# iliasam/STM32F4_SDR_GPS

Hardware: AMD Instinct MI355X
Metric: acquisition hypotheses/sec (PRN x Doppler x phase) (higher is better)
Workload: dtype u1 (MX-FP4 operands, exact f32 accumulation)

## Files before the change

### stm32f4_sdr_gps_amd/csrc/k_acq_mx.hip

```cpp
#if !defined(GPSX_LAB) && defined(MX_VARIANT_B)
#error "variants of k_acq_mx for same-box A/B timing build with -DGPSX_LAB only: tools/build_variant.sh"
#endif
#include <cstdlib>

#include "gpsx_device.hpp"
#include "gpsx_kernels.hpp"

namespace gpsx {

namespace {

typedef int v8i __attribute__((ext_vector_type(8)));
typedef int v4i __attribute__((ext_vector_type(4)));
typedef float v16f __attribute__((ext_vector_type(16)));

constexpr int kMxThreads = 512;
constexpr int kMxTiles = 4;
constexpr int kCopyDwords = 260;
constexpr int kVecDwords = 258;
constexpr int kPlaneWordsMx = 66;
constexpr u32 kScaleOne = 0x7F7F7F7Fu;
constexpr u32 kScaleA = 0x72727272u;
constexpr float kAccScale = 1.0f / 8192.0f;
constexpr float kUnscaleSq = 67108864.0f;
constexpr u32 kScaleEight = 0x82828282u;
constexpr int kPasses = 17;

struct MxShared {
  uint16_t x[1024];
  u32 d[2][514];
  u32 plane[2][16][kPlaneWordsMx];
  u32 base[2][kCopyDwords];
  u32 e8[2][2][8][kCopyDwords];
  u32 corr[2][2][2][128];
  v4i chips_a[16][2][32];
  u32 chip_t[1032];
  u32 ones[2];
  u32 t_lut[768];
  alignas(16) u32 part[8][32][2][32];
};

__device__ __forceinline__ v8i widen(v4i x) { return v8i{x.x, x.y, x.z, x.w, 0, 0, 0, 0}; }

__device__ __forceinline__ u32 lds_byte(const u32 *words, int byte_index)
{
  return (words[byte_index >> 2] >> ((byte_index & 3) * 8)) & 0xFFu;
}

__device__ __forceinline__ u32 spread8(u32 x)
{
  u32 t = (x | (x << 12)) & 0x000F000Fu;
  t = (t | (t << 6)) & 0x03030303u;
  t = (t | (t << 3)) & 0x11111111u;
  return t;
}

__device__ __forceinline__ int wrap1023(int i)
{
  i = i >= 2 * kChips ? i - 2 * kChips : i;
  return i >= kChips ? i - kChips : i;
}

__device__ __forceinline__ u32 plane_bits9(const u32 *pl, int pos)
{
  return __builtin_amdgcn_alignbit(pl[(pos >> 5) + 1], pl[pos >> 5], (u32)(pos & 31)) & 0x1FFu;
}

__device__ __forceinline__ void mx_load_block(MxShared &sh, const uint8_t *blk, int if_format, int tid)
{
  for (int i = tid; i < 1024; i += kMxThreads)
    sh.x[i] = i < kWords16 ? load_sign16(blk, i, if_format) : (uint16_t)0;
  if (tid < 2)
    sh.ones[tid] = 0;
}
__device__ void mx_wipe_block(MxShared &sh, u32 step_word, int tid, int lane)
{
  {
    const u32 *x32 = reinterpret_cast<const u32 *>(sh.x);
    u32 ones_i = 0, ones_q = 0;
    for (int w = tid; w < 514; w += kMxThreads) {
      u32 vi = 0, vq = 0;
      if (w < kWords32) {
        const u32 quad = (step_word * (u32)w) >> 30;
        vi = carrier_i(quad) ^ x32[w];
        vq = carrier_q(quad) ^ x32[w];
      }
      sh.d[0][w] = vi;
      sh.d[1][w] = vq;
      ones_i += __popc(vi);
      ones_q += __popc(vq);
    }
    ones_i = wave_sum_to_lane63(ones_i);
    ones_q = wave_sum_to_lane63(ones_q);
    if (lane == 63) {
      atomicAdd(&sh.ones[0], ones_i);
      atomicAdd(&sh.ones[1], ones_q);
    }
  }
  __syncthreads();
  if (tid < 2)
    sh.d[tid][511] = sh.d[tid][0] << 16;
  __syncthreads();
  for (int m = tid; m < 2 * 32 * 16; m += kMxThreads) {
    const int t0 = m & 15, w = (m >> 4) & 31, iq = m >> 9;
    const u32 *src = &sh.d[iq][16 * w];
    u32 bits = 0;
#pragma unroll
    for (int k = 0; k < 16; k++) {
      const u32 sk = src[k];
      bits |= ((sk >> t0) & 1u) << (2 * k);
      bits |= ((sk >> (16 + t0)) & 1u) << (2 * k + 1);
    }
    sh.plane[iq][t0][w] = bits;
  }
  __syncthreads();
  for (int m = tid; m < 2 * 16 * (kPlaneWordsMx - 32); m += kMxThreads) {
    const int w = 32 + m % (kPlaneWordsMx - 32);
    const int r = m / (kPlaneWordsMx - 32);
    const u32 *pl = sh.plane[r >> 4][r & 15];
    const int pos = 32 * w - (w >= 64 ? 2 * kChips : kChips);
    const int lo = pos >> 5;
    u32 v = __builtin_amdgcn_alignbit(lo < 31 ? pl[lo + 1] : 0u, pl[lo], (u32)(pos & 31));
    if (pos + 32 > kChips) {
      const int k = kChips - pos;
      v = (v & ((1u << k) - 1u)) | (pl[0] << k);
    }
    sh.plane[r >> 4][r & 15][w] = v;
  }
}

__device__ __forceinline__ u32 fp4_code(int v)
{
  const u32 m = (u32)(v < 0 ? -v : v);
  return ((0x0765420u >> (4u * (m > 5u ? 5u : m))) & 0xFu) | (v < 0 ? 8u : 0u);
}

__device__ void mx_fill_tables(MxShared &sh, int tid)
{
  for (int w = tid; w < 512; w += kMxThreads) {
    const u32 cur = (u32)w & 0xFFu, nxt = ((u32)w >> 1) & 0xFFu;
    const u32 plus = spread8(nxt & ~cur), minus = spread8(cur & ~nxt);
    sh.t_lut[w] = (plus << 2) | (plus << 3) | (minus << 2);
  }
  for (int x = tid; x < 256; x += kMxThreads)
    sh.t_lut[512 + x] = (spread8((u32)x) << 1) | (spread8(~(u32)x & 0xFFu) * 0xAu);
}

__device__ void mx_vector_phase1(MxShared &sh, int pass, int buf, int tid, int nthreads)
{
  const int t0 = pass - 1;
  for (int m = tid; m < 2 * kVecDwords + 2 * 128; m += nthreads) {
    if (m < 2 * kVecDwords) {
      const int iq = m >= kVecDwords, dw = m - iq * kVecDwords;
      u32 packed = 0;
      if (pass < 2) {
        const u32 *dd = sh.d[iq];
#pragma unroll
        for (int e = 0; e < 8; e++) {
          const int k = wrap1023(8 * dw + e);
          const int pos = 16 * k;
          const u32 sum = pop16(__builtin_amdgcn_alignbit(dd[(pos >> 5) + 1], dd[pos >> 5], (u32)(pos & 31)));
          const u32 code = pass == 0 ? (0xFEC0u >> (4u * (sum & 3u))) & 0xFu : (0xEDCA0u >> (4u * (sum >> 2))) & 0xFu;
          packed |= code << (4 * e);
        }
      } else {
        const u32 w = plane_bits9(sh.plane[iq][pass - 2], 8 * dw);
        packed = sh.t_lut[w];
        if (dw == 127 && t0 >= 9) {
          const u32 cur = w & 0xFFu, nxt = (w >> 1) & 0xFFu;
          const int e5 = (int)((nxt >> 5) & 1u) - (int)((cur >> 5) & 1u), e6 = (int)((nxt >> 6) & 1u) - (int)((cur >> 6) & 1u);
          packed = (packed & ~0x0FF00000u) | (fp4_code(-2 * e5 - 1) << 20) | (fp4_code(-2 * e6 + 1) << 24);
        }
      }
      sh.base[iq][dw] = packed;
    } else {
      const int mm = m - 2 * kVecDwords;
      const int iq = mm >> 7, dw = mm & 127;
      u32 ca = 0, cb = 0;
      if (pass >= 2 && t0 != 8) {
        const u32 *pl = sh.plane[iq][pass - 2];
        const u32 w = dw ? plane_bits9(pl, 8 * dw - 1) : (pl[0] << 1) & 0x1FFu;
        const u32 exist = dw == 127 ? 0x0FFFFFFFu : 0xFFFFFFFFu;
        if (t0 < 8) {
          ca = sh.t_lut[512 + (w >> 1)] & exist;
        } else {
          const u32 diff = sh.t_lut[w];
          ca = (diff ^ ((diff & 0x44444444u) << 1)) & exist;
          cb = sh.t_lut[512 + (w & 0xFFu)] & exist;
          if (dw == 0) {
            ca = (ca & ~0xFu) | ((w & 2u) ? 0x2u : 0xAu);
            cb &= ~0xFu;
          }
        }
      }
      sh.corr[buf][iq][0][dw] = ca;
      sh.corr[buf][iq][1][dw] = cb;
    }
  }
}

__device__ void mx_vector_phase2(MxShared &sh, int buf, int tid, int nthreads)
{
  for (int m = tid; m < 2 * 256; m += nthreads) {
    const int iq = m >> 8, j = m & 255;
    const u32 lo = sh.base[iq][j], hi = sh.base[iq][j + 1];
#pragma unroll
    for (int c = 0; c < 8; c++)
      sh.e8[buf][iq][c][j] = c ? __builtin_amdgcn_alignbit(hi, lo, 4u * (u32)c) : lo;
  }
}

typedef __attribute__((address_space(3))) const u32 lds_cu32;

__device__ __forceinline__ lds_cu32 *lds_opaque(const u32 *p)
{
  u32 a = (u32)(size_t)(lds_cu32 *)p;
  asm volatile("" : "+v"(a));
  return (lds_cu32 *)(size_t)a;
}
__device__ __forceinline__ v4i lds_frag(lds_cu32 *w, int dw)
{
  return v4i{(int)w[dw], (int)w[dw + 1], (int)w[dw + 2], (int)w[dw + 3]};
}

__device__ __forceinline__ u32 mx_patch_wrap(u32 packed, u32 w9, bool patch)
{
  const u32 i5 = 1u + ((w9 >> 6) & 1u) - ((w9 >> 5) & 1u), i6 = 1u + ((w9 >> 7) & 1u) - ((w9 >> 6) & 1u);
  const u32 c5 = (0xDA2u >> (4u * i5)) & 0xFu;
  const u32 c6 = (0xA25u >> (4u * i6)) & 0xFu;
  const u32 patched = (packed & ~0x0FF00000u) | (c5 << 20) | (c6 << 24);
  return patch ? patched : packed;
}

__device__ __forceinline__ void mx_vector_build(MxShared &sh, int p_vec, int tid)
{
  const int t0 = p_vec - 1, buf = p_vec & 1;
  const bool late = t0 >= 9;
  const int iq = tid >> 8, j = tid & 255, which = (tid >> 7) & 1, dwc = tid & 127;
  const u32 *pl = sh.plane[iq][p_vec - 2];
  const u32 x = __builtin_amdgcn_alignbit(pl[(j >> 2) + 1], pl[j >> 2], 8u * (u32)(j & 3));
  const int pos = dwc ? 8 * dwc - 1 : 0;
  const u32 y = __builtin_amdgcn_alignbit(pl[(pos >> 5) + 1], pl[pos >> 5], (u32)(pos & 31));
  const u32 cw = (dwc ? y : y << 1) & 0x1FFu;
  u32 lo = sh.t_lut[x & 0x1FFu], hi = sh.t_lut[(x >> 8) & 0x1FFu];
  u32 v = sh.t_lut[which ? 512u + (cw & 0xFFu) : (late ? cw : 512u + (cw >> 1))];
  if (late) {
    lo = mx_patch_wrap(lo, x & 0x1FFu, j == 127);
    hi = mx_patch_wrap(hi, (x >> 8) & 0x1FFu, j == 126);
    if (which == 0)
      v ^= (v & 0x44444444u) << 1;
    if (dwc == 0)
      v = (v & ~0xFu) | (which ? 0u : ((cw & 2u) ? 0x2u : 0xAu));
  }
  v &= dwc == 127 ? 0x0FFFFFFFu : 0xFFFFFFFFu;
  if ((which && !late) || t0 == 8)
    v = 0;
  sh.corr[buf][iq][which][dwc] = v;
  u32 *dst = &sh.e8[buf][iq][0][j];
#pragma unroll
  for (int c = 0; c < 8; c++)
    dst[c * kCopyDwords] = c ? __builtin_amdgcn_alignbit(hi, lo, 4u * (u32)c) : lo;
}

__device__ __forceinline__ void mx_vector_build_direct(MxShared &sh, int which, int t0s, u32 *e8_dst, int tid)
{
  const int iq = tid >> 8, j = tid & 255;
  const u32 *dd = sh.d[iq];
  u32 w2[2] = {0, 0};
#pragma unroll
  for (int e = 0; e < 16; e++) {
    const int k = wrap1023(8 * j + e);
    const int pos = 16 * k + t0s;
    const u32 sum = pop16(__builtin_amdgcn_alignbit(dd[(pos >> 5) + 1], dd[pos >> 5], (u32)(pos & 31)));
    const u32 code = which == 0 ? (0xFEC0u >> (4u * (sum & 3u))) & 0xFu : (0xEDCA0u >> (4u * (sum >> 2))) & 0xFu;
    w2[e >> 3] |= code << (4 * (e & 7));
  }
  u32 *dst = e8_dst + (iq * 8) * kCopyDwords + j;
#pragma unroll
  for (int c = 0; c < 8; c++)
    dst[c * kCopyDwords] = c ? __builtin_amdgcn_alignbit(w2[1], w2[0], 4u * (u32)c) : w2[0];
}

template <int S, int NT, u32 SCALE_A = kScaleA>
__device__ __forceinline__ void mx_pass_step(lds_cu32 *wi, lds_cu32 *wq, const v4i *ca, v4i (&a)[16], v4i &fi, v4i &fq,
                                             v16f (&acc)[2][NT], u32 scale_b)
{
  constexpr int kSteps = 16 + NT - 1;
  constexpr bool more = S + 1 < kSteps;
  v4i fi_next = fi, fq_next = fq;
  if constexpr (more) {
    fi_next = lds_frag(wi, 8 * (S + 1));
    fq_next = lds_frag(wq, 8 * (S + 1));
    if constexpr (S + 1 < 16)
      a[S + 1] = ca[(S + 1) * 64];
  }
  constexpr int j_lo = S - 15 > 0 ? S - 15 : 0, j_hi = S < NT - 1 ? S : NT - 1;
#pragma unroll
  for (int j = j_lo; j <= j_hi; j++) {
    acc[0][j] = __builtin_amdgcn_mfma_scale_f32_32x32x64_f8f6f4(widen(a[S - j]), widen(fi), acc[0][j], 4, 4, 0, SCALE_A, 0, scale_b);
    acc[1][j] = __builtin_amdgcn_mfma_scale_f32_32x32x64_f8f6f4(widen(a[S - j]), widen(fq), acc[1][j], 4, 4, 0, SCALE_A, 0, scale_b);
  }
  if constexpr (more) {
    __builtin_amdgcn_sched_group_barrier(0x100, S + 1 < 16 ? 5 : 4, 0);
    __builtin_amdgcn_sched_group_barrier(0x008, 2 * (j_hi - j_lo + 1), 0);
  }
  __builtin_amdgcn_sched_barrier(0);
  fi = fi_next;
  fq = fq_next;
  if constexpr (more)
    mx_pass_step<S + 1, NT, SCALE_A>(wi, wq, ca, a, fi, fq, acc, scale_b);
}

template <int S, int NT>
__device__ __forceinline__ void mx_pass_step_inplace(lds_cu32 *wi, lds_cu32 *wq, const v4i *ca, v4i (&a)[16], v4i &fi, v4i &fq,
                                                     v16f (&acc)[2][NT], u32 scale_b)
{
  constexpr int kSteps = 16 + NT - 1;
  constexpr bool more = S + 1 < kSteps;
  if constexpr (more && S + 1 < 16)
    a[S + 1] = ca[(S + 1) * 64];
  constexpr int j_lo = S - 15 > 0 ? S - 15 : 0, j_hi = S < NT - 1 ? S : NT - 1;
#pragma unroll
  for (int j = j_lo; j <= j_hi; j++)
    acc[0][j] = __builtin_amdgcn_mfma_scale_f32_32x32x64_f8f6f4(widen(a[S - j]), widen(fi), acc[0][j], 4, 4, 0, kScaleA, 0, scale_b);
  if constexpr (more)
    fi = lds_frag(wi, 8 * (S + 1));
#pragma unroll
  for (int j = j_lo; j <= j_hi; j++)
    acc[1][j] = __builtin_amdgcn_mfma_scale_f32_32x32x64_f8f6f4(widen(a[S - j]), widen(fq), acc[1][j], 4, 4, 0, kScaleA, 0, scale_b);
  if constexpr (more)
    fq = lds_frag(wq, 8 * (S + 1));
  if constexpr (more) {
    if constexpr (S + 1 < 16)
      __builtin_amdgcn_sched_group_barrier(0x100, 1, 0);
    __builtin_amdgcn_sched_group_barrier(0x008, j_hi - j_lo + 1, 0);
    __builtin_amdgcn_sched_group_barrier(0x100, 2, 0);
    __builtin_amdgcn_sched_group_barrier(0x008, j_hi - j_lo + 1, 0);
    __builtin_amdgcn_sched_group_barrier(0x100, 2, 0);
  }
  __builtin_amdgcn_sched_barrier(0);
  if constexpr (more)
    mx_pass_step_inplace<S + 1, NT>(wi, wq, ca, a, fi, fq, acc, scale_b);
}

template <int S, int NT>
__device__ __forceinline__ void mx_pass2_step(lds_cu32 *const (&w)[4], const v4i *ca, v4i (&a)[16], v4i (&f)[4], v16f (&acc)[2][NT])
{
  constexpr int kSteps = 16 + NT - 1;
  constexpr bool more = S + 1 < kSteps;
  if constexpr (more && S + 1 < 16)
    a[S + 1] = ca[(S + 1) * 64];
  constexpr int j_lo = S - 15 > 0 ? S - 15 : 0, j_hi = S < NT - 1 ? S : NT - 1;
#pragma unroll
  for (int v = 0; v < 4; v++) {
#pragma unroll
    for (int j = j_lo; j <= j_hi; j++)
      acc[v & 1][j] = __builtin_amdgcn_mfma_scale_f32_32x32x64_f8f6f4(widen(a[S - j]), widen(f[v]), acc[v & 1][j], 4, 4, 0, kScaleA, 0,
                                                                      v < 2 ? kScaleOne : kScaleEight);
    if constexpr (more)
      f[v] = lds_frag(w[v], 8 * (S + 1));
  }
  if constexpr (more) {
    if constexpr (S + 1 < 16)
      __builtin_amdgcn_sched_group_barrier(0x100, 1, 0);
#pragma unroll
    for (int v = 0; v < 4; v++) {
      __builtin_amdgcn_sched_group_barrier(0x008, j_hi - j_lo + 1, 0);
      __builtin_amdgcn_sched_group_barrier(0x100, 2, 0);
    }
  }
  __builtin_amdgcn_sched_barrier(0);
  if constexpr (more)
    mx_pass2_step<S + 1, NT>(w, ca, a, f, acc);
}
template <int NT>
__device__ __forceinline__ void mx_pass2(const MxShared &sh, int lane, int q0_tile, v16f (&acc)[2][NT], const u32 *e8_low,
                                         const u32 *e8_high)
{
  const int n = lane & 31, h = lane >> 5;
  const int off = (n & 7) * kCopyDwords + 4 * (q0_tile + h) + (n >> 3);
  lds_cu32 *const w[4] = {lds_opaque(e8_low + off), lds_opaque(e8_low + 8 * kCopyDwords + off), lds_opaque(e8_high + off),
                          lds_opaque(e8_high + 8 * kCopyDwords + off)};
  const v4i *ca = &sh.chips_a[0][h][n];
  v4i a[16];
  v4i f[4] = {lds_frag(w[0], 0), lds_frag(w[1], 0), lds_frag(w[2], 0), lds_frag(w[3], 0)};
  a[0] = ca[0];
  mx_pass2_step<0, NT>(w, ca, a, f, acc);
}

template <bool AHEAD, int NT, u32 SCALE_A = kScaleA>
__device__ __forceinline__ void mx_pass(const MxShared &sh, int buf, int lane, int q0_tile, v16f (&acc)[2][NT],
                                        u32 scale_b, v4i a_corr, bool with_corr, const u32 *e8_buf = nullptr)
{
  const int n = lane & 31, h = lane >> 5;
  const u32 *e8 = e8_buf ? e8_buf : &sh.e8[buf][0][0][0];
  lds_cu32 *wi = lds_opaque(e8 + (n & 7) * kCopyDwords + 4 * (q0_tile + h) + (n >> 3));
  lds_cu32 *wq = lds_opaque(e8 + (8 + (n & 7)) * kCopyDwords + 4 * (q0_tile + h) + (n >> 3));
  const v4i *ca = &sh.chips_a[0][h][n];
  v4i a[16];
  if constexpr (AHEAD) {
    v4i fi = lds_frag(wi, 0), fq = lds_frag(wq, 0);
    a[0] = ca[0];
    mx_pass_step<0, NT, SCALE_A>(wi, wq, ca, a, fi, fq, acc, scale_b);
  } else {
    static_assert(SCALE_A == kScaleA, "the in-place walk is the sign-only grid's");
    v4i fi = lds_frag(wi, 0), fq = lds_frag(wq, 0);
    a[0] = ca[0];
    mx_pass_step_inplace<0, NT>(wi, wq, ca, a, fi, fq, acc, scale_b);
  }
  if (with_corr) {
    lds_cu32 *cw = lds_opaque(&sh.corr[buf][0][h][4 * q0_tile + (n >> 3)]);
#pragma unroll
    for (int j = 0; j < NT; j++) {
      const v4i gi = v4i{(int)(cw[8 * j] >> (4 * (n & 7))), 0, 0, 0};
      const v4i gq = v4i{(int)(cw[8 * j + 2 * 128] >> (4 * (n & 7))), 0, 0, 0};
      acc[0][j] = __builtin_amdgcn_mfma_scale_f32_32x32x64_f8f6f4(widen(a_corr), widen(gi), acc[0][j], 4, 4, 0, kScaleA, 0,
                                                                   kScaleOne);
      acc[1][j] = __builtin_amdgcn_mfma_scale_f32_32x32x64_f8f6f4(widen(a_corr), widen(gq), acc[1][j], 4, 4, 0, kScaleA, 0,
                                                                   kScaleOne);
    }
  }
}

__device__ __forceinline__ u32 root_trunc(float e);
__device__ __forceinline__ float mx_clip_square(float c)
{
  return __builtin_amdgcn_fmed3f(c * __builtin_fabsf(c), 0.0f, 1.0f);
}
__device__ __forceinline__ float clip_square_sum(float ci, float cq)
{
  return mx_clip_square(ci) + mx_clip_square(cq);
}
__device__ __forceinline__ u32 mag8_f32(float ci, float cq)
{
  return root_trunc(clip_square_sum(ci, cq) * kUnscaleSq);
}

__device__ __forceinline__ u32 root_trunc(float e)
{
  float r = __builtin_amdgcn_sqrtf(e);
  const float r_dn = __uint_as_float(__float_as_uint(r) - 1u);
  const float r_up = __uint_as_float(__float_as_uint(r) + 1u);
  const float res_dn = __builtin_fmaf(-r_dn, r, e);
  const float res_up = __builtin_fmaf(-r_up, r, e);
  r = res_dn <= 0.0f ? r_dn : r;
  r = res_up > 0.0f ? r_up : r;
  return (u32)(int)r;
}

constexpr float kRootGuard = 8192.001953125f;
__device__ __forceinline__ void mx_round_toward_zero()
{
  asm volatile("s_setreg_imm32_b32 hwreg(HW_REG_MODE, 0, 2), 3\n\ts_nop 1" ::: "memory");
  __builtin_amdgcn_sched_barrier(0);
}
__device__ __forceinline__ void mx_round_to_nearest()
{
  __builtin_amdgcn_sched_barrier(0);
  asm volatile("s_setreg_imm32_b32 hwreg(HW_REG_MODE, 0, 2), 0\n\ts_nop 1" ::: "memory");
}
__device__ __forceinline__ u32 root_bits_small(float e)
{
  return __float_as_uint(__builtin_fmaf(__builtin_amdgcn_sqrtf(e), kRootGuard, 8388608.0f));
}
template <int N>
__device__ __forceinline__ void mx_roots_exact(float (&ci)[N], float (&cq)[N], u32 (&mag)[N])
{
  static_assert(N == 4 || N == 8, "group size");
  if constexpr (N == 8)
    asm volatile("s_setreg_imm32_b32 hwreg(HW_REG_MODE, 0, 2), 0\n\ts_nop 1"
                 : "+v"(ci[0]), "+v"(ci[1]), "+v"(ci[2]), "+v"(ci[3]), "+v"(ci[4]), "+v"(ci[5]), "+v"(ci[6]), "+v"(ci[7]),
                   "+v"(cq[0]), "+v"(cq[1]), "+v"(cq[2]), "+v"(cq[3]), "+v"(cq[4]), "+v"(cq[5]), "+v"(cq[6]), "+v"(cq[7]));
  else
    asm volatile("s_setreg_imm32_b32 hwreg(HW_REG_MODE, 0, 2), 0\n\ts_nop 1"
                 : "+v"(ci[0]), "+v"(ci[1]), "+v"(ci[2]), "+v"(ci[3]), "+v"(cq[0]), "+v"(cq[1]), "+v"(cq[2]), "+v"(cq[3]));
#pragma unroll
  for (int i = 0; i < N; i++)
    mag[i] = mag8_f32(ci[i], cq[i]);
  if constexpr (N == 8)
    asm volatile("s_setreg_imm32_b32 hwreg(HW_REG_MODE, 0, 2), 3\n\ts_nop 1"
                 : "+v"(mag[0]), "+v"(mag[1]), "+v"(mag[2]), "+v"(mag[3]), "+v"(mag[4]), "+v"(mag[5]), "+v"(mag[6]), "+v"(mag[7]));
  else
    asm volatile("s_setreg_imm32_b32 hwreg(HW_REG_MODE, 0, 2), 3\n\ts_nop 1"
                 : "+v"(mag[0]), "+v"(mag[1]), "+v"(mag[2]), "+v"(mag[3]));
}

constexpr float kOutside = -1048576.0f * kAccScale;

template <int NT>
__device__ __forceinline__ void mx_init_acc(const u32 *ones, int lane, int q0_tile, v16f (&acc)[2][NT], int win_start,
                                            int win_stop)
{
  const int n = lane & 31;
  const float base_i = (float)((int)ones[0] + 8192 - kHalf) * kAccScale, base_q = (float)((int)ones[1] + 8192 - kHalf) * kAccScale;
#pragma unroll
  for (int j = 0; j < NT; j++) {
    const int q = 32 * (q0_tile + 2 * j) + n;
    const int o = 2 * q;
    const bool in_win = q < kChips && o >= win_start && o < win_stop;
#pragma unroll
    for (int r = 0; r < 16; r++) {
      acc[0][j][r] = in_win ? base_i : base_i + kOutside;
      acc[1][j][r] = in_win ? base_q : base_q + kOutside;
    }
  }
}

template <int NT>
__device__ __forceinline__ void mx_half_switch(const MxShared &sh, int lane, int q0_tile, v16f (&acc)[2][NT], int win_start,
                                               int win_stop)
{
  const int n = lane & 31, h = lane >> 5;
  const u32 *d_i = sh.d[0], *d_q = sh.d[1];
  const u32 wrap_i = (d_i[0] & 0xFFu) << 8, wrap_q = (d_q[0] & 0xFFu) << 8;
  const float beta0_i = (float)(16 - 2 * (int)__popc(wrap_i)) * kAccScale, beta0_q = (float)(16 - 2 * (int)__popc(wrap_q)) * kAccScale;
  const int popw_i = (int)__popc(wrap_i), popw_q = (int)__popc(wrap_q);
  const u32 f22 = sh.chip_t[1022 + 1] >> (4 * h);
#pragma unroll
  for (int j = 0; j < NT; j++) {
    const int q = 32 * (q0_tile + 2 * j) + n;
    const bool exists = q < kChips;
    const int qc = exists ? q : 0;
    const bool in0 = exists && 2 * q >= win_start && 2 * q < win_stop;
    const bool in1 = exists && 2 * q + 1 >= win_start && 2 * q + 1 < win_stop;
    int fa_i = -(2 * (int)__popc(lds_byte(d_i, 2 * qc) & 0x7Fu) - 7);
    int fa_q = -(2 * (int)__popc(lds_byte(d_q, 2 * qc) & 0x7Fu) - 7);
    int fk_i = -popw_i, fk_q = -popw_q;
    if (q > 0 && exists) {
      const u32 prev_i = lds_byte(d_i, 2 * qc - 1) | (lds_byte(d_i, 2 * qc) << 8);
      const u32 prev_q = lds_byte(d_q, 2 * qc - 1) | (lds_byte(d_q, 2 * qc) << 8);
      fk_i -= (int)__popc(prev_i);
      fk_q -= (int)__popc(prev_q);
      fa_i -= 16 - 2 * (int)__popc(prev_i);
      fa_q -= 16 - 2 * (int)__popc(prev_q);
    }
    float fkf_i = (float)fk_i * kAccScale, fkf_q = (float)fk_q * kAccScale;
    if (in0 != in1) {
      fkf_i += in1 ? -kOutside : kOutside;
      fkf_q += in1 ? -kOutside : kOutside;
    }
    const float faf_i = (float)fa_i * kAccScale, faf_q = (float)fa_q * kAccScale;
    const u32 w1 = sh.chip_t[(exists ? kChips - 1 - q : 0) + 1] >> (4 * h);
#pragma unroll
    for (int r = 0; r < 16; r++) {
      const int pb = (r & 3) + 8 * (r >> 2);
      const float c22 = (float)((f22 >> pb) & 1u), c1 = (float)((w1 >> pb) & 1u);
      acc[0][j][r] += fkf_i + c22 * faf_i - c1 * beta0_i;
      acc[1][j][r] += fkf_q + c22 * faf_q - c1 * beta0_q;
    }
  }
}

template <int NT>
// ... 363 lines not shown
          bits[i] += kRootBias;
      }
#pragma unroll
      for (int rr = 0; rr < 4; rr++) {
        const int r = r0 + rr;
        const u32 k0 = (bits[rr] << 11) | kqh[jp], k1 = (bits[4 + rr] << 11) | kqh[jp + 1];
        best[r] = max(max(best[r], k0), k1);
        total[r] = total[r] + bits[rr] + bits[4 + rr];
      }
#pragma unroll
      for (int rr = 0; rr < 4; rr++)
        asm volatile("" : "+v"(best[r0 + rr]), "+v"(total[r0 + rr]));
      __builtin_amdgcn_sched_barrier(0);
    }
  }
  mx_round_to_nearest();
#pragma unroll
  for (int r = 0; r < 16; r++) {
    const int p_off = ((r & 3) + 8 * (r >> 2)) * 64;
    atomicMax(slot + p_off, best[r]);
    atomicAdd(slot + p_off + 32, total[r]);
  }
}

__device__ __forceinline__ void mx_epilogue_store(int lane, int q0_tile, int t0, const v16f (&acc)[2][kMxTiles], u32 group_mask,
                                                  uint16_t *__restrict__ plane0, size_t prn_stride, int slot0, int n_prn)
{
  const int n = lane & 31, h = lane >> 5;
#pragma unroll
  for (int j = 0; j < kMxTiles; j++) {
    const int q = 32 * (q0_tile + 2 * j) + n;
    uint16_t *v = plane0 + (size_t)t0 * 1024 + (size_t)(q & 3) * 256 + (size_t)(q >> 2);
#pragma unroll
    for (int g = 0; g < 4; g++) {
#pragma unroll
      for (int rr = 0; rr < 4; rr++) {
        const int r = 4 * g + rr;
        const int p = (r & 3) + 8 * (r >> 2) + 4 * h;
        const u32 val = mag8_f32(acc[0][j][r], acc[1][j][r]);
        if (((group_mask >> g) & 1u) && slot0 + p < n_prn)
          v[(size_t)p * prn_stride] = (uint16_t)val;
      }
      __builtin_amdgcn_sched_barrier(0);
    }
  }
}



__device__ __forceinline__ unsigned long long mx_max8_u64(unsigned long long v)
{
  u32 lo = (u32)v, hi = (u32)(v >> 32);
#define MX_MAX8(ctrl)                                                                           \
  {                                                                                             \
    const u32 lo2 = (u32)__builtin_amdgcn_mov_dpp((int)lo, ctrl, 0xF, 0xF, true);               \
    const u32 hi2 = (u32)__builtin_amdgcn_mov_dpp((int)hi, ctrl, 0xF, 0xF, true);               \
    const bool g = hi2 > hi || (hi2 == hi && lo2 > lo);                                         \
    lo = g ? lo2 : lo;                                                                          \
    hi = g ? hi2 : hi;                                                                          \
  }
  MX_MAX8(0xB1)
  MX_MAX8(0x4E)
  MX_MAX8(0x141)
#undef MX_MAX8
  return ((unsigned long long)hi << 32) | lo;
}

constexpr int kMxSingle = 0, kMxWalk = 1, kMxStore = 2, kMxWalk16 = 3, kMxByte = 4, kMxSplit = 5;

}

__global__ void k_build_mx_tables(const u32 *__restrict__ chipbits, int n_slots, u32 *__restrict__ mx_a, u32 *__restrict__ mx_t)
{
  const int n_sets = (n_slots + 31) / 32;
  const int idx = blockIdx.x * blockDim.x + threadIdx.x;
  const int per_set = 16 * 2 * 32 * 4 + 1032;
  if (idx >= n_sets * per_set)
    return;
  const int set = idx / per_set, r = idx - set * per_set;
  if (r < 16 * 2 * 32 * 4) {
    const int dw = r & 3, p = (r >> 2) & 31, h = (r >> 7) & 1, kappa = r >> 8;
    const int slot = 32 * set + p;
    const u32 word = slot < n_slots ? chipbits[(size_t)slot * 32 + 2 * kappa + h] : 0u;
    mx_a[(size_t)set * (16 * 2 * 32 * 4) + r] = spread8((word >> (8 * dw)) & 0xFFu) << 1;
  } else {
    const int c = r - 16 * 2 * 32 * 4 - 1;
    u32 w = 0;
    if (c >= 0 && c < kChips)
      for (int p = 0; p < 32; p++) {
        const int slot = 32 * set + p;
        if (slot < n_slots)
          w |= ((chipbits[(size_t)slot * 32 + (c >> 5)] >> (c & 31)) & 1u) << p;
      }
    mx_t[(size_t)set * 1032 + (c + 1)] = w;
  }
}

void launch_build_mx_tables(hipStream_t s, const uint32_t *d_chipbits, int n_slots, uint32_t *d_mx_a, uint32_t *d_mx_t)
{
  const int n_sets = (n_slots + 31) / 32;
  const int n = n_sets * (16 * 2 * 32 * 4 + 1032);
  hipLaunchKernelGGL(k_build_mx_tables, dim3((n + 255) / 256), dim3(256), 0, s, d_chipbits, n_slots, d_mx_a, d_mx_t);
}

template <int MODE>
__device__ __forceinline__ void mx_unit(MxShared &sh, const AcqParams &prm, int wg, int &tables_set, int cluster_lo,
                                        const uint8_t *__restrict__ if_blocks, const u32 *__restrict__ mx_a,
                                        const u32 *__restrict__ mx_t, gpsx_peak_t *__restrict__ peaks, u32 *__restrict__ energy,
                                        u32 *__restrict__ flags)
{
  constexpr bool MULTI = MODE == kMxWalk || MODE == kMxWalk16, STORE = MODE == kMxStore, S16 = MODE == kMxWalk16;
  constexpr bool SPLIT = MODE == kMxSplit;
  typedef SumRecT<S16> SumRec;
  if constexpr (MODE == kMxWalk) {
    if (flags && flags[wg] == 0)
      return;
  }
  const int tid = threadIdx.x;
  const int lane = tid & 63, wave = __builtin_amdgcn_readfirstlane(tid >> 6);
  const int role = wave >> 2;
  const int q0_tile = 8 * (wave >> 1) + (wave & 1);

  const int n_sets = (prm.n_groups + 3) / 4;
  const int ms_store = STORE ? wg % prm.n_ms : 0;
  const int n_seg = SPLIT ? prm.split_segs : 1;
  const int seg = SPLIT ? wg % n_seg : 0;
  const int cluster = cluster_lo + (STORE ? wg / prm.n_ms : SPLIT ? wg / n_seg : wg);
  const int set = cluster % n_sets;
  const int sd = cluster / n_sets;
  const int dopp = sd % prm.n_dopp;
  const int search = sd / prm.n_dopp;
  u32 group_mask = 0;
#pragma unroll
  for (int g = 0; g < 4; g++) {
    const int group = 4 * set + g;
    const int unit = sd * prm.n_groups + group;
    if (group < prm.n_groups && unit >= prm.unit_lo && unit < prm.unit_hi)
      group_mask |= 1u << g;
  }
  group_mask = (u32)__builtin_amdgcn_readfirstlane((int)group_mask);
  if (group_mask == 0)
    return;
  const float freq_hz = (float)(prm.if_hz + prm.dopp_min_hz + dopp * prm.dopp_step_hz);
  const u32 step_word = nco_step_per_word(freq_hz);

  if (tables_set != set) {
    const u32 *src_a = mx_a + (size_t)set * (16 * 2 * 32 * 4);
    u32 *dst_a = reinterpret_cast<u32 *>(&sh.chips_a[0][0][0]);
    for (int i = tid; i < 16 * 2 * 32 * 4; i += kMxThreads)
      dst_a[i] = src_a[i];
    const u32 *src_t = mx_t + (size_t)set * 1032;
    for (int i = tid; i < 1032; i += kMxThreads)
      sh.chip_t[i] = src_t[i];
    mx_fill_tables(sh, tid);
    tables_set = set;
  }
  for (int i = tid; i < 8 * 32 * 2 * 32 / 4; i += kMxThreads)
    reinterpret_cast<uint4 *>(&sh.part[0][0][0][0])[i] = make_uint4(0, 0, 0, 0);
  const size_t block_bytes = prm.if_format == GPSX_IF_2BIT_SM ? GPSX_BYTES_PER_MS_2BIT : kBytes;
  const uint8_t *block0 = if_blocks + (size_t)(search * prm.search_stride_blocks + (STORE ? wg % prm.n_ms : 0)) * block_bytes;
  mx_load_block(sh, block0, prm.if_format, tid);

  __syncthreads();
  const v4i a_corr = v4i{(int)(((sh.chip_t[(lane >> 5 ? 1021 : 1022) + 1] >> (lane & 31)) & 1u) << 1), 0, 0, 0};
  u32 kq[kMxTiles];
#pragma unroll
  for (int j = 0; j < kMxTiles; j++) {
    kq[j] = (u32)(2047 - 2 * (32 * (q0_tile + 2 * j) + (lane & 31)));
    if constexpr (!MULTI && !STORE)
      asm volatile("" : "+v"(kq[j]));
  }
  u32 *e_wave = MULTI ? energy + ((size_t)wg * 8 + wave) * (16 * kMxTiles * 4 * 64 * (S16 ? 2 : 3)) : nullptr;
  const u32 *zero_recs = MULTI ? flags - kMxZeroRecBytes / sizeof(u32) : nullptr;
  u32 witness = 0;
  const int n_ms = MULTI ? prm.n_ms : 1;
  const int t0s = SPLIT ? seg * (16 / n_seg) : 0;
  const int n_pass = SPLIT ? 16 / n_seg + 1 : kPasses;
  const int pbase = t0s;
#pragma unroll 1
  for (int ms = 0; ms < n_ms; ms++) {
    const bool ms_first = ms == 0, ms_last = ms == n_ms - 1;
    int tid_p = tid, lane_p = lane;
    if constexpr (MULTI)
      asm volatile("" : "+v"(tid_p), "+v"(lane_p));
    if (ms > 0) {
      __syncthreads();
      mx_load_block(sh, block0 + (size_t)ms * block_bytes, prm.if_format, tid_p);
      __syncthreads();
    }
    mx_wipe_block(sh, step_word, tid_p, lane_p);
    if (SPLIT && seg) {
      mx_vector_build_direct(sh, 0, t0s, &sh.e8[0][0][0][0], tid);
      mx_vector_build_direct(sh, 1, t0s, &sh.e8[1][0][0][0], tid);
      for (int i = tid; i < 2 * 2 * 2 * 128; i += kMxThreads)
        (&sh.corr[0][0][0][0])[i] = 0;
    } else {
      __syncthreads();
      mx_vector_phase1(sh, 0, 0, tid_p, kMxThreads);
      __syncthreads();
      mx_vector_phase2(sh, 0, tid_p, kMxThreads);
      __syncthreads();
      mx_vector_phase1(sh, 1, 1, tid_p, kMxThreads);
      __syncthreads();
      mx_vector_phase2(sh, 1, tid_p, kMxThreads);
    }

    v16f acc[2][kMxTiles];
    mx_init_acc(sh.ones, lane_p, q0_tile, acc, prm.win_start, prm.win_stop);
    SumRec pre[MULTI ? 16 : 1];

#pragma unroll 1
    for (int hs = 0; hs <= 2 * n_pass; hs++) {
      if ((hs & 1) == 0)
        __syncthreads();
      constexpr bool kBuildBehindEpilogue = MULTI;
      if (!kBuildBehindEpilogue && (hs & 1) == 0) {
        const int p_vec = (hs >> 1) + 1;
        if (p_vec >= 2 && p_vec < n_pass) {
          int tid_v = tid;
          if constexpr (MULTI)
            asm volatile("" : "+v"(tid_v));
          mx_vector_build(sh, pbase + p_vec, tid_v);
        }
      }
      int lane_s = lane;
      if constexpr (MULTI)
        asm volatile("" : "+v"(lane_s));
      const int x = hs - role;
      const bool active = x >= 0 && x < 2 * n_pass;
      const int p = x >> 1;
      if (active && (x & 1) == 0) {
        if constexpr (MULTI) {
          if (p >= 1)
            mx_prefetch_sums<0, 8, S16>(e_wave, zero_recs, lane_s, p - 1, ms_first, pre);
        }
        mx_pass<!MULTI>(sh, p & 1, lane, q0_tile, acc, p == 1 ? kScaleEight : kScaleOne, a_corr, p >= 2 && (SPLIT || p != 9));
        if constexpr (SPLIT) {
          if (p == 1 && seg) {
            int lane_d = lane;
            asm volatile("" : "+v"(lane_d));
            mx_direct_terms(sh, lane_d, q0_tile, acc, t0s, prm.win_start, prm.win_stop);
          }
        } else {
          if (p == 9)
            mx_half_switch(sh, lane_s, q0_tile, acc, prm.win_start, prm.win_stop);
        }
      }
      if (STORE) {
        if (active && (x & 1) && p >= 1) {
          uint16_t *plane0 = reinterpret_cast<uint16_t *>(energy) +
                             ((size_t)((search * prm.n_ms + ms_store) * prm.n_prn + 32 * set) * prm.n_dopp + dopp) * (16 * 1024);
          mx_epilogue_store(lane, q0_tile, p - 1, acc, group_mask, plane0, (size_t)prm.n_dopp * (16 * 1024), 32 * set, prm.n_prn);
        }
      } else if (active && (x & 1) && p >= 1) {
        if (!MULTI)
          mx_epilogue_single(sh, lane, kq, t0s + p - 1, acc);
        else if (!ms_last)
          mx_epilogue<MULTI, false, S16>(sh, lane_s, q0_tile, p - 1, acc, group_mask, e_wave, zero_recs, pre, ms_first, witness);
        else
          mx_epilogue<MULTI, true, S16>(sh, lane_s, q0_tile, p - 1, acc, group_mask, e_wave, zero_recs, pre, ms_first, witness);
      }
      if (kBuildBehindEpilogue && (x & 1) != 0) {
        const int p_vec = (hs >> 1) + 1;
        if (p_vec >= 2 && p_vec < n_pass) {
          int tid_v = tid;
          if constexpr (MULTI)
            asm volatile("" : "+v"(tid_v));
          mx_vector_build(sh, pbase + p_vec, tid_v);
        }
      }
    }
  }
  if (STORE)
    return;
  if constexpr (S16) {
    if (tid == 0)
      sh.ones[0] = 0;
    __syncthreads();
    if (__builtin_amdgcn_ballot_w64(witness >= 0xFFFFu) != 0 && lane == 0)
      atomicOr(&sh.ones[0], 1u);
  }
  __syncthreads();
  if constexpr (S16) {
    if (tid == 0)
      flags[wg] = sh.ones[0];
    if (sh.ones[0])
      return;
  }
  {
    const int which = tid >> 8, p = (tid >> 3) & 31, b = tid & 7;
    const int slot = 32 * set + p;
    const u32 *row = sh.part[b][p][which];
    u32 vals[32];
#pragma unroll
    for (int l = 0; l < 32; l++)
      vals[l] = row[(l + tid) & 31];
    u32 k = 0, t = 0;
#pragma unroll
    for (int l = 0; l < 32; l++) {
      k = vals[l] > k ? vals[l] : k;
      t += vals[l];
    }
    if (((group_mask >> (p >> 3)) & 1u) && slot < prm.n_prn && b < prm.n_bits) {
      const size_t idx = ((size_t)(search * prm.n_prn + slot) * prm.n_dopp + dopp) * prm.n_bits + b;
      uint2 *pk = reinterpret_cast<uint2 *>(&peaks[idx]);
      if constexpr (SPLIT) {
        const size_t n_planes = (size_t)prm.n_planes;
        if (which == 0)
          atomicMax(&energy[idx], k);
        else
          atomicAdd(&energy[n_planes + idx], t);
      } else if (which == 0) {
        const u32 max_val = k >> 11;
        pk[0] = make_uint2(max_val, max_val ? 2047u - (k & 2047u) : 0u);
      } else {
        pk[1] = make_uint2(t, t / (2u * kChips));
      }
    }
    if constexpr (!SPLIT) {
      if (prm.keys && which == 0) {
        unsigned long long key = 0;
        if (b < prm.n_bits) {
          const u32 max_val = k >> 11, phase = max_val ? 2047u - (k & 2047u) : 0u;
          key = ((unsigned long long)max_val << 14) | (unsigned long long)(16383u - (8u * phase + (u32)b));
        }
        key = mx_max8_u64(key);
        if (b == 0 && ((group_mask >> (p >> 3)) & 1u) && slot < prm.n_prn)
          prm.keys[(size_t)(search * prm.n_prn + slot) * prm.n_dopp + dopp] = (int64_t)key;
      }
    }
  }
}

struct MxBlockRegs {
  u32 v[4];
};
__device__ __forceinline__ MxBlockRegs mx_block_request(const uint8_t *blk, int if_format, int tid)
{
  MxBlockRegs r;
  const uint16_t *p = reinterpret_cast<const uint16_t *>(blk);
  const bool second = 2 * tid + 1 < kWords16;
  if (if_format == GPSX_IF_2BIT_SM) {
    r.v[0] = p[4 * tid];
    r.v[1] = p[4 * tid + 1];
    r.v[2] = second ? p[4 * tid + 2] : 0;
    r.v[3] = second ? p[4 * tid + 3] : 0;
  } else {
    r.v[0] = p[2 * tid];
    r.v[1] = second ? p[2 * tid + 1] : 0;
    r.v[2] = r.v[3] = 0;
  }
  return r;
}
__device__ __forceinline__ void mx_block_commit(MxShared &sh, const MxBlockRegs &r, int if_format, int tid)
{
  u32 lo = r.v[0], hi = r.v[1];
  if (if_format == GPSX_IF_2BIT_SM) {
    lo = even_bits16(r.v[0] | (r.v[1] << 16));
    hi = even_bits16(r.v[2] | (r.v[3] << 16));
  }
  reinterpret_cast<u32 *>(sh.x)[tid] = (lo & 0xFFFFu) | (hi << 16);
}

__device__ __forceinline__ u32 sum_code_low(u32 s) { return (0xFEC0u >> ((s << 2) & 0xCu)) & 0xFu; }
__device__ __forceinline__ u32 sum_code_high(u32 s) { return (0xEDCA0u >> (s & 0x1Cu)) & 0xFu; }

__device__ __forceinline__ void mx_byte_fill_code_table(MxShared &sh, int tid)
{
  uint16_t *lut = reinterpret_cast<uint16_t *>(sh.t_lut);
  static_assert(sizeof(sh.t_lut) >= 1024 * sizeof(uint16_t), "code table fits");
  for (int i = tid; i < 1024; i += kMxThreads) {
    const u32 sa = (u32)i & 31u, sb = (u32)i >> 5;
    lut[i] = (uint16_t)(sum_code_low(sa) | (sum_code_low(sb) << 4) | (sum_code_high(sa) << 8) | (sum_code_high(sb) << 12));
  }
}

__device__ __forceinline__ void mx_byte_wipe_codes(const MxShared &sh, u32 *d, u32 *ones, u32 *base0, u32 *base8, u32 step_word,
                                                   int tid, int lane)
{
  const u32 *x32 = reinterpret_cast<const u32 *>(sh.x);
  const uint16_t *lut = reinterpret_cast<const uint16_t *>(sh.t_lut);
  const int w = tid, k = tid & 3;
  const u32 x_first = x32[0], x_cur = x32[w], x_next = x32[w < 511 ? w + 1 : 0];
  const u32 quad_cur = (step_word * (u32)w) >> 30, quad_next = (step_word * (u32)(w + 1)) >> 30;
  const u32 sel = (u32)k * 0x0101u + 0x0400u;
  const int item_dword = (k & 1) * 258 + (k >> 1) * 128 + (w >> 2);
  u32 cnt = 0;
#pragma unroll
  for (int s = 0; s < 2; s++) {
    const u32 first = (s ? carrier_q(0u) : carrier_i(0u)) ^ x_first;
    const u32 wrap = first << 16;
    const u32 cur = w < kWords32 ? (s ? carrier_q(quad_cur) : carrier_i(quad_cur)) ^ x_cur : wrap;
    const u32 nxt = w + 1 < kWords32 ? (s ? carrier_q(quad_next) : carrier_i(quad_next)) ^ x_next : (w + 1 == kWords32 ? wrap : 0u);
    d[s * 514 + w] = cur;
    cnt += (w < kWords32 ? (u32)__popc(cur) : 0u) << (16 * s);
    const u32 x8 = __builtin_amdgcn_alignbit(nxt, cur, 8u);
#pragma unroll
    for (int o = 0; o < 2; o++) {
      u32 s0 = pop16(o ? x8 : cur), s1 = (u32)__popc((o ? x8 : cur) >> 16);
      const u32 s2 = pop16(o ? nxt >> 8 : nxt);
      if (o && w == 511) {
        s1 = pop16(first >> 8);
        s0 = 8;
      }
      const u32 pk = (u32)lut[s0 | (s1 << 5)] | ((u32)lut[s1 | (s2 << 5)] << 16);
      u32 *base = (o ? base8 : base0) + s * (2 * 258);
      const u32 p0 = (u32)__builtin_amdgcn_mov_dpp((int)pk, 0x00, 0xF, 0xF, true), p1 = (u32)__builtin_amdgcn_mov_dpp((int)pk, 0x55, 0xF, 0xF, true);
      const u32 p2 = (u32)__builtin_amdgcn_mov_dpp((int)pk, 0xAA, 0xF, 0xF, true), p3 = (u32)__builtin_amdgcn_mov_dpp((int)pk, 0xFF, 0xF, 0xF, true);
      const u32 out = (__builtin_amdgcn_perm(p1, p0, sel) & 0xFFFFu) | (__builtin_amdgcn_perm(p3, p2, sel) << 16);
      if (w < 508 || k < 2)
        base[item_dword] = out;
      uint8_t *bytes = reinterpret_cast<uint8_t *>(base);
      if (w >= 508 && w < 511) {
        bytes[512 + w] = (uint8_t)(pk >> 16);
        bytes[258 * 4 + 512 + w] = (uint8_t)(pk >> 24);
      }
      if (w < 5) {
        bytes[1023 + w] = (uint8_t)pk;
        bytes[258 * 4 + 1023 + w] = (uint8_t)(pk >> 8);
      }
    }
// ... 884 lines not shown
```

Before: 1323 billion.

## Fold wrap-around correction into last K-step operand patch for single-ms path

For the non-MULTI path, the separate correction MFMA term (extra K step using corr vectors and a_corr) is replaced by patching the top nibbles of the final B fragment per tile from a precomputed per-position patch table. A small p_lut is built at table fill, and mx_vector_build writes shifted patch words into a union aliasing the old corr storage. This removes the extra correction K-step and the corr zeroing, at the cost of extra LDS reads and bit-masking inside the MFMA step chain, plus a changed scheduling group count.

After: 1333 billion (median of 6 runs). No clear change (+0.8%).

```diff
diff --git a/stm32f4_sdr_gps_amd/csrc/k_acq_mx.hip b/stm32f4_sdr_gps_amd/csrc/k_acq_mx.hip
--- a/stm32f4_sdr_gps_amd/csrc/k_acq_mx.hip
+++ b/stm32f4_sdr_gps_amd/csrc/k_acq_mx.hip
@@ -32,11 +32,15 @@
   u32 plane[2][16][kPlaneWordsMx];
   u32 base[2][kCopyDwords];
   u32 e8[2][2][8][kCopyDwords];
-  u32 corr[2][2][2][128];
+  union {
+    u32 patch[2][1024][2];
+    u32 corr[2][2][2][128];
+  };
   v4i chips_a[16][2][32];
   u32 chip_t[1032];
   u32 ones[2];
   u32 t_lut[768];
+  u32 p_lut[3][64];
   alignas(16) u32 part[8][32][2][32];
 };
 
@@ -135,7 +139,7 @@
   return ((0x0765420u >> (4u * (m > 5u ? 5u : m))) & 0xFu) | (v < 0 ? 8u : 0u);
 }
 
-__device__ void mx_fill_tables(MxShared &sh, int tid)
+__device__ void mx_fill_tables(MxShared &sh, int tid, bool with_patches)
 {
   for (int w = tid; w < 512; w += kMxThreads) {
     const u32 cur = (u32)w & 0xFFu, nxt = ((u32)w >> 1) & 0xFFu;
@@ -144,58 +148,45 @@
   }
   for (int x = tid; x < 256; x += kMxThreads)
     sh.t_lut[512 + x] = (spread8((u32)x) << 1) | (spread8(~(u32)x & 0xFFu) * 0xAu);
-}
-
-__device__ void mx_vector_phase1(MxShared &sh, int pass, int buf, int tid, int nthreads)
+  for (int x = tid; with_patches && x < 3 * 64; x += kMxThreads) {
+    const int kind = x >> 6;
+    u32 m = 0;
+    for (int i = 0; i < 4; i++) {
+      const int g0 = (x >> i) & 1, g1 = (x >> (i + 1)) & 1, g2 = (x >> (i + 2)) & 1;
+      const int r1021 = kind < 2 ? -2 * (g1 - g0) : 2 * g0 - 1;
+      const int r1022 = kind == 0 ? 2 * g1 - 1 : kind == 1 ? -2 * (g2 - g1) : 0;
+      m |= (fp4_code(r1021) | (fp4_code(r1022) << 4)) << (8 * i);
+    }
+    sh.p_lut[kind][x & 63] = m;
+  }
+}
+
+__device__ void mx_vector_phase1(MxShared &sh, int pass, int tid, int nthreads)
 {
   const int t0 = pass - 1;
-  for (int m = tid; m < 2 * kVecDwords + 2 * 128; m += nthreads) {
-    if (m < 2 * kVecDwords) {
-      const int iq = m >= kVecDwords, dw = m - iq * kVecDwords;
-      u32 packed = 0;
-      if (pass < 2) {
-        const u32 *dd = sh.d[iq];
-#pragma unroll
-        for (int e = 0; e < 8; e++) {
-          const int k = wrap1023(8 * dw + e);
-          const int pos = 16 * k;
-          const u32 sum = pop16(__builtin_amdgcn_alignbit(dd[(pos >> 5) + 1], dd[pos >> 5], (u32)(pos & 31)));
-          const u32 code = pass == 0 ? (0xFEC0u >> (4u * (sum & 3u))) & 0xFu : (0xEDCA0u >> (4u * (sum >> 2))) & 0xFu;
-          packed |= code << (4 * e);
-        }
-      } else {
-        const u32 w = plane_bits9(sh.plane[iq][pass - 2], 8 * dw);
-        packed = sh.t_lut[w];
-        if (dw == 127 && t0 >= 9) {
-          const u32 cur = w & 0xFFu, nxt = (w >> 1) & 0xFFu;
-          const int e5 = (int)((nxt >> 5) & 1u) - (int)((cur >> 5) & 1u), e6 = (int)((nxt >> 6) & 1u) - (int)((cur >> 6) & 1u);
-          packed = (packed & ~0x0FF00000u) | (fp4_code(-2 * e5 - 1) << 20) | (fp4_code(-2 * e6 + 1) << 24);
-        }
-      }
-      sh.base[iq][dw] = packed;
+  for (int m = tid; m < 2 * kVecDwords; m += nthreads) {
+    const int iq = m >= kVecDwords, dw = m - iq * kVecDwords;
+    u32 packed = 0;
+    if (pass < 2) {
+      const u32 *dd = sh.d[iq];
+#pragma unroll
+      for (int e = 0; e < 8; e++) {
+        const int k = wrap1023(8 * dw + e);
+        const int pos = 16 * k;
+        const u32 sum = pop16(__builtin_amdgcn_alignbit(dd[(pos >> 5) + 1], dd[pos >> 5], (u32)(pos & 31)));
+        const u32 code = pass == 0 ? (0xFEC0u >> (4u * (sum & 3u))) & 0xFu : (0xEDCA0u >> (4u * (sum >> 2))) & 0xFu;
+        packed |= code << (4 * e);
+      }
     } else {
-      const int mm = m - 2 * kVecDwords;
-      const int iq = mm >> 7, dw = mm & 127;
-      u32 ca = 0, cb = 0;
-      if (pass >= 2 && t0 != 8) {
-        const u32 *pl = sh.plane[iq][pass - 2];
-        const u32 w = dw ? plane_bits9(pl, 8 * dw - 1) : (pl[0] << 1) & 0x1FFu;
-        const u32 exist = dw == 127 ? 0x0FFFFFFFu : 0xFFFFFFFFu;
-        if (t0 < 8) {
-          ca = sh.t_lut[512 + (w >> 1)] & exist;
-        } else {
-          const u32 diff = sh.t_lut[w];
-          ca = (diff ^ ((diff & 0x44444444u) << 1)) & exist;
-          cb = sh.t_lut[512 + (w & 0xFFu)] & exist;
-          if (dw == 0) {
-            ca = (ca & ~0xFu) | ((w & 2u) ? 0x2u : 0xAu);
-            cb &= ~0xFu;
-          }
-        }
-      }
-      sh.corr[buf][iq][0][dw] = ca;
-      sh.corr[buf][iq][1][dw] = cb;
-    }
+      const u32 w = plane_bits9(sh.plane[iq][pass - 2], 8 * dw);
+      packed = sh.t_lut[w];
+      if (dw == 127 && t0 >= 9) {
+        const u32 cur = w & 0xFFu, nxt = (w >> 1) & 0xFFu;
+        const int e5 = (int)((nxt >> 5) & 1u) - (int)((cur >> 5) & 1u), e6 = (int)((nxt >> 6) & 1u) - (int)((cur >> 6) & 1u);
+        packed = (packed & ~0x0FF00000u) | (fp4_code(-2 * e5 - 1) << 20) | (fp4_code(-2 * e6 + 1) << 24);
+      }
+    }
+    sh.base[iq][dw] = packed;
   }
 }
 
@@ -211,6 +202,8 @@
 }
 
 typedef __attribute__((address_space(3))) const u32 lds_cu32;
+typedef u32 v2u __attribute__((ext_vector_type(2)));
+typedef __attribute__((address_space(3))) const v2u lds_cv2u;
 
 __device__ __forceinline__ lds_cu32 *lds_opaque(const u32 *p)
 {
@@ -232,30 +225,50 @@
   return patch ? patched : packed;
 }
 
+template <bool FOLD>
 __device__ __forceinline__ void mx_vector_build(MxShared &sh, int p_vec, int tid)
 {
   const int t0 = p_vec - 1, buf = p_vec & 1;
   const bool late = t0 >= 9;
-  const int iq = tid >> 8, j = tid & 255, which = (tid >> 7) & 1, dwc = tid & 127;
+  const int iq = tid >> 8, j = tid & 255;
   const u32 *pl = sh.plane[iq][p_vec - 2];
   const u32 x = __builtin_amdgcn_alignbit(pl[(j >> 2) + 1], pl[j >> 2], 8u * (u32)(j & 3));
-  const int pos = dwc ? 8 * dwc - 1 : 0;
-  const u32 y = __builtin_amdgcn_alignbit(pl[(pos >> 5) + 1], pl[pos >> 5], (u32)(pos & 31));
-  const u32 cw = (dwc ? y : y << 1) & 0x1FFu;
   u32 lo = sh.t_lut[x & 0x1FFu], hi = sh.t_lut[(x >> 8) & 0x1FFu];
-  u32 v = sh.t_lut[which ? 512u + (cw & 0xFFu) : (late ? cw : 512u + (cw >> 1))];
   if (late) {
     lo = mx_patch_wrap(lo, x & 0x1FFu, j == 127);
     hi = mx_patch_wrap(hi, (x >> 8) & 0x1FFu, j == 126);
-    if (which == 0)
-      v ^= (v & 0x44444444u) << 1;
-    if (dwc == 0)
-      v = (v & ~0xFu) | (which ? 0u : ((cw & 2u) ? 0x2u : 0xAu));
-  }
-  v &= dwc == 127 ? 0x0FFFFFFFu : 0xFFFFFFFFu;
-  if ((which && !late) || t0 == 8)
-    v = 0;
-  sh.corr[buf][iq][which][dwc] = v;
+  }
+  if constexpr (FOLD) {
+    const int pos = 4 * j + 1021;
+    const u32 g = __builtin_amdgcn_alignbit(pl[(pos >> 5) + 1], pl[pos >> 5], (u32)(pos & 31)) & 0x3Fu;
+    u32 m = sh.p_lut[t0 < 8 ? 0 : t0 == 8 ? 1 : 2][g];
+    if (late && j == 0) {
+      const u32 c5 = (0xDA2u >> (4u * (1u + ((g >> 1) & 1u) - (g & 1u)))) & 0xFu;
+      const u32 two_d = (g & 2u) << 1;
+      m = (m & 0xFFFF0000u) | c5 | (two_d << 4) | (two_d << 8);
+    }
+    u32 *dst = &sh.patch[buf][4 * j][iq];
+    dst[0] = m << 20;
+    dst[2] = m << 12;
+    dst[4] = m << 4;
+    dst[6] = m >> 4;
+  } else {
+    const int which = (tid >> 7) & 1, dwc = tid & 127;
+    const int pos = dwc ? 8 * dwc - 1 : 0;
+    const u32 y = __builtin_amdgcn_alignbit(pl[(pos >> 5) + 1], pl[pos >> 5], (u32)(pos & 31));
+    const u32 cw = (dwc ? y : y << 1) & 0x1FFu;
+    u32 v = sh.t_lut[which ? 512u + (cw & 0xFFu) : (late ? cw : 512u + (cw >> 1))];
+    if (late) {
+      if (which == 0)
+        v ^= (v & 0x44444444u) << 1;
+      if (dwc == 0)
+        v = (v & ~0xFu) | (which ? 0u : ((cw & 2u) ? 0x2u : 0xAu));
+    }
+    v &= dwc == 127 ? 0x0FFFFFFFu : 0xFFFFFFFFu;
+    if ((which && !late) || t0 == 8)
+      v = 0;
+    sh.corr[buf][iq][which][dwc] = v;
+  }
   u32 *dst = &sh.e8[buf][iq][0][j];
 #pragma unroll
   for (int c = 0; c < 8; c++)
@@ -281,12 +294,14 @@
     dst[c * kCopyDwords] = c ? __builtin_amdgcn_alignbit(w2[1], w2[0], 4u * (u32)c) : w2[0];
 }
 
-template <int S, int NT, u32 SCALE_A = kScaleA>
+template <int S, int NT, u32 SCALE_A = kScaleA, bool FOLD = false>
 __device__ __forceinline__ void mx_pass_step(lds_cu32 *wi, lds_cu32 *wq, const v4i *ca, v4i (&a)[16], v4i &fi, v4i &fq,
-                                             v16f (&acc)[2][NT], u32 scale_b)
+                                             v16f (&acc)[2][NT], u32 scale_b, lds_cv2u *pw = nullptr, u32 pmask = 0,
+                                             v2u *pt = nullptr)
 {
   constexpr int kSteps = 16 + NT - 1;
   constexpr bool more = S + 1 < kSteps;
+  constexpr bool patch_read = FOLD && S >= 12 && S - 12 < NT;
   v4i fi_next = fi, fq_next = fq;
   if constexpr (more) {
     fi_next = lds_frag(wi, 8 * (S + 1));
@@ -294,21 +309,28 @@
     if constexpr (S + 1 < 16)
       a[S + 1] = ca[(S + 1) * 64];
   }
+  if constexpr (patch_read)
+    pt[S - 12] = pw[64 * (S - 12)];
   constexpr int j_lo = S - 15 > 0 ? S - 15 : 0, j_hi = S < NT - 1 ? S : NT - 1;
 #pragma unroll
-  for (int j = j_lo; j <= j_hi; j++) {
+  for (int k = 0; k <= j_hi - j_lo; k++) {
+    const int j = FOLD ? j_hi - k : j_lo + k;
+    if (FOLD && S - j == 15) {
+      fi.w = (int)(((u32)fi.w & ~pmask) | (pt[j].x & pmask));
+      fq.w = (int)(((u32)fq.w & ~pmask) | (pt[j].y & pmask));
+    }
     acc[0][j] = __builtin_amdgcn_mfma_scale_f32_32x32x64_f8f6f4(widen(a[S - j]), widen(fi), acc[0][j], 4, 4, 0, SCALE_A, 0, scale_b);
     acc[1][j] = __builtin_amdgcn_mfma_scale_f32_32x32x64_f8f6f4(widen(a[S - j]), widen(fq), acc[1][j], 4, 4, 0, SCALE_A, 0, scale_b);
   }
   if constexpr (more) {
-    __builtin_amdgcn_sched_group_barrier(0x100, S + 1 < 16 ? 5 : 4, 0);
+    __builtin_amdgcn_sched_group_barrier(0x100, (S + 1 < 16 ? 5 : 4) + (patch_read ? 1 : 0), 0);
     __builtin_amdgcn_sched_group_barrier(0x008, 2 * (j_hi - j_lo + 1), 0);
   }
   __builtin_amdgcn_sched_barrier(0);
   fi = fi_next;
   fq = fq_next;
   if constexpr (more)
-    mx_pass_step<S + 1, NT, SCALE_A>(wi, wq, ca, a, fi, fq, acc, scale_b);
+    mx_pass_step<S + 1, NT, SCALE_A, FOLD>(wi, wq, ca, a, fi, fq, acc, scale_b, pw, pmask, pt);
 }
 
 template <int S, int NT>
@@ -388,7 +410,7 @@
   mx_pass2_step<0, NT>(w, ca, a, f, acc);
 }
 
-template <bool AHEAD, int NT, u32 SCALE_A = kScaleA>
+template <bool AHEAD, int NT, u32 SCALE_A = kScaleA, bool FOLD = false>
 __device__ __forceinline__ void mx_pass(const MxShared &sh, int buf, int lane, int q0_tile, v16f (&acc)[2][NT],
                                         u32 scale_b, v4i a_corr, bool with_corr, const u32 *e8_buf = nullptr)
 {
@@ -398,7 +420,16 @@
   lds_cu32 *wq = lds_opaque(e8 + (8 + (n & 7)) * kCopyDwords + 4 * (q0_tile + h) + (n >> 3));
   const v4i *ca = &sh.chips_a[0][h][n];
   v4i a[16];
-  if constexpr (AHEAD) {
+  static_assert(AHEAD || !FOLD, "the in-place walk keeps the extra K step");
+  if constexpr (FOLD) {
+    lds_cv2u *pw = (lds_cv2u *)lds_opaque(&sh.patch[buf][32 * q0_tile + n][0]);
+    const u32 pmask = h && with_corr ? 0x0FF00000u : 0u;
+    v2u pt[NT];
+    v4i fi = lds_frag(wi, 0), fq = lds_frag(wq, 0);
+    a[0] = ca[0];
+    mx_pass_step<0, NT, SCALE_A, true>(wi, wq, ca, a, fi, fq, acc, scale_b, pw, pmask, pt);
+    return;
+  } else if constexpr (AHEAD) {
     v4i fi = lds_frag(wi, 0), fq = lds_frag(wq, 0);
     a[0] = ca[0];
     mx_pass_step<0, NT, SCALE_A>(wi, wq, ca, a, fi, fq, acc, scale_b);
@@ -1068,7 +1099,7 @@
     const u32 *src_t = mx_t + (size_t)set * 1032;
     for (int i = tid; i < 1032; i += kMxThreads)
       sh.chip_t[i] = src_t[i];
-    mx_fill_tables(sh, tid);
+    mx_fill_tables(sh, tid, !MULTI);
     tables_set = set;
   }
   for (int i = tid; i < 8 * 32 * 2 * 32 / 4; i += kMxThreads)
@@ -1078,7 +1109,9 @@
   mx_load_block(sh, block0, prm.if_format, tid);
 
   __syncthreads();
-  const v4i a_corr = v4i{(int)(((sh.chip_t[(lane >> 5 ? 1021 : 1022) + 1] >> (lane & 31)) & 1u) << 1), 0, 0, 0};
+  v4i a_corr = v4i{0, 0, 0, 0};
+  if constexpr (MULTI)
+    a_corr.x = (int)(((sh.chip_t[(lane >> 5 ? 1021 : 1022) + 1] >> (lane & 31)) & 1u) << 1);
   u32 kq[kMxTiles];
 #pragma unroll
   for (int j = 0; j < kMxTiles; j++) {
@@ -1108,15 +1141,13 @@
     if (SPLIT && seg) {
       mx_vector_build_direct(sh, 0, t0s, &sh.e8[0][0][0][0], tid);
       mx_vector_build_direct(sh, 1, t0s, &sh.e8[1][0][0][0], tid);
-      for (int i = tid; i < 2 * 2 * 2 * 128; i += kMxThreads)
-        (&sh.corr[0][0][0][0])[i] = 0;
     } else {
       __syncthreads();
-      mx_vector_phase1(sh, 0, 0, tid_p, kMxThreads);
+      mx_vector_phase1(sh, 0, tid_p, kMxThreads);
       __syncthreads();
       mx_vector_phase2(sh, 0, tid_p, kMxThreads);
       __syncthreads();
-      mx_vector_phase1(sh, 1, 1, tid_p, kMxThreads);
+      mx_vector_phase1(sh, 1, tid_p, kMxThreads);
       __syncthreads();
       mx_vector_phase2(sh, 1, tid_p, kMxThreads);
     }
@@ -1136,7 +1167,7 @@
           int tid_v = tid;
           if constexpr (MULTI)
             asm volatile("" : "+v"(tid_v));
-          mx_vector_build(sh, pbase + p_vec, tid_v);
+          mx_vector_build<!MULTI>(sh, pbase + p_vec, tid_v);
         }
       }
       int lane_s = lane;
@@ -1150,7 +1181,8 @@
           if (p >= 1)
             mx_prefetch_sums<0, 8, S16>(e_wave, zero_recs, lane_s, p - 1, ms_first, pre);
         }
-        mx_pass<!MULTI>(sh, p & 1, lane, q0_tile, acc, p == 1 ? kScaleEight : kScaleOne, a_corr, p >= 2 && (SPLIT || p != 9));
+        mx_pass<!MULTI, kMxTiles, kScaleA, !MULTI>(sh, p & 1, lane, q0_tile, acc, p == 1 ? kScaleEight : kScaleOne, a_corr,
+                                                   p >= 2 && (!MULTI || p != 9));
         if constexpr (SPLIT) {
           if (p == 1 && seg) {
             int lane_d = lane;
@@ -1182,7 +1214,7 @@
           int tid_v = tid;
           if constexpr (MULTI)
             asm volatile("" : "+v"(tid_v));
-          mx_vector_build(sh, pbase + p_vec, tid_v);
+          mx_vector_build<!MULTI>(sh, pbase + p_vec, tid_v);
         }
       }
     }
```
